# sdu-hpcl/BGSA

Hardware: AMD Instinct MI355X
Metric: GCUPS (cell updates/sec) all-pairs Myers 150bp (higher is better)
Workload: dtype u32

## Files before the change

bgsa_amd/__init__.py:

```python
from __future__ import annotations

import ctypes
import os
import subprocess
from pathlib import Path

import numpy as np

HERE = Path(__file__).resolve().parent
LIB_PATH = Path(os.environ["BGSA_HIP_LIB"]) if os.environ.get("BGSA_HIP_LIB") else HERE / "libbgsa_hip.so"
LIB_AB_PATH = HERE / "libbgsa_hip_ab.so"
INCLUDE = HERE.parent / "include" / "bgsa_hip.h"

ALGO_MYERS, ALGO_BANDED, ALGO_BITPAL = 0, 1, 2
DISTANCE_BEYOND = -2
V_NUM = 64

_lib = None


class Params(ctypes.Structure):
    _fields_ = [("algo", ctypes.c_int), ("alignment", ctypes.c_int), ("match", ctypes.c_int),
                ("mismatch", ctypes.c_int), ("gap", ctypes.c_int), ("k", ctypes.c_int)]

# ... 79 lines not shown
    L.bgsa_hip_bucket_resident.argtypes = [vp, sz, i32]
    L.bgsa_hip_bucket_release.argtypes = [vp]
    u64p = ctypes.POINTER(ctypes.c_uint64)
    L.bgsa_hip_seam_stats.argtypes = [u64p, u64p, u64p]
    L.bgsa_hip_row_cache_stats.argtypes = [u64p, u64p]
    L.bgsa_hip_event_create.argtypes = [ctypes.POINTER(vp)]
    L.bgsa_hip_event_destroy.argtypes = [vp]
    L.bgsa_hip_event_record.argtypes = [vp, vp]
    L.bgsa_hip_event_synchronize.argtypes = [vp]
    L.bgsa_hip_event_elapsed_ms.argtypes = [vp, vp, ctypes.POINTER(ctypes.c_float)]
    L.bgsa_hip_stream_wait_event.argtypes = [vp, vp]
    L.bgsa_hip_query_stream.argtypes = [i32, vp, i32, i32, vp, i32]
    L.bgsa_hip_myers_band_stream.argtypes = [vp, i32, i32, vp, i32]
    L.bgsa_hip_myers_band_half.argtypes = [i32, i32]
    L.bgsa_hip_myers_band_stats.argtypes = [vp, i32]
    L.bgsa_hip_kernel_name.argtypes = [i32, i32]
    L.bgsa_hip_kernel_name.restype = ctypes.c_char_p
    L.bgsa_hip_malloc.argtypes = [ctypes.POINTER(vp), sz]
    L.bgsa_hip_free.argtypes = [vp]
    L.bgsa_hip_malloc_host.argtypes = [ctypes.POINTER(vp), sz]
    L.bgsa_hip_free_host.argtypes = [vp]
    L.bgsa_hip_memcpy_h2d.argtypes = [vp, vp, sz, vp]
    L.bgsa_hip_memcpy_d2h.argtypes = [vp, vp, sz, vp]
    L.bgsa_hip_memset.argtypes = [vp, i32, sz, vp]
    L.bgsa_hip_stream_synchronize.argtypes = [vp]
    L.bgsa_hip_stream_create.argtypes = [ctypes.POINTER(vp)]
    L.bgsa_hip_stream_destroy.argtypes = [vp]
    L.bgsa_hip_set_device.argtypes = [i32]
    L.hip_handle_reads.argtypes = [vp, vp, i32, i64, i64]
    L.hip_handle_reads.restype = None
# ... 544 lines not shown
```

bgsa_amd/csrc/bgsa_common.h:

```cpp
#pragma once

#include <hip/hip_runtime.h>
#include <stdint.h>
#include <stdlib.h>
#include <stdio.h>

#include <type_traits>

#include "../../include/bgsa_hip.h"

namespace bgsa {

constexpr int kLanes = HIP_V_NUM;
constexpr int kChars = BGSA_CHAR_NUM;
constexpr int kWavesPerBlock = 4;
constexpr int kMaxWords = 32;

void set_error(const char *what, hipError_t e, const char *file, int line);
void set_error_text(const char *text);

#define BGSA_HIP_TRY(expr)                                              \
    do {                                                                \
        hipError_t e_ = (expr);                                         \
        if (e_ != hipSuccess) {                                         \
// ... 46 lines not shown
        if (((N == nw ? (rc = f(std::integral_constant<int, N>{}), true) : false) || ...)) return rc;
        char msg[128];
        snprintf(msg, sizeof msg, "%s: no kernel of %d words in this build", family, nw);
        set_error_text(msg);
        return BGSA_HIP_EUNSUPPORTED;
    }
    template <int M>
    constexpr Widths<N..., M> with() const { return {}; }
};
template <typename A, typename B> struct JoinWidths;
template <int... A, int... B> struct JoinWidths<Widths<A...>, Widths<B...>> { using type = Widths<A..., B...>; };
template <typename A, typename B> using Join = typename JoinWidths<A, B>::type;

int launch_myers(const ScoreArgs &a, int semi_global = 0);
const char *myers_kernel_name(int word_num, int semi_global = 0);

constexpr int kCodeEnd = 5, kCodeRefill = 6;
inline int stream_windows(int ref_len) { return ref_len / 7 + 1; }
inline size_t stream_stride(int ref_len) { return static_cast<size_t>(stream_windows(ref_len) + 1) * 8; }
__host__ __device__ inline unsigned long long plain_stream_window(const char *row, int ref_len, int i)
{
    const int n_windows = ref_len / 7 + 1;
    unsigned long long win = 0;
    for (int j = 0; j < 8; j++) {
        unsigned code = kCodeEnd;
        if (i < n_windows) {
            const int pos = 7 * i + j;
            if (j == 7) code = (i < n_windows - 1) ? kCodeRefill : kCodeEnd;
            else if (pos < ref_len) {
                code = static_cast<unsigned char>(row[pos]);
// ... 432 lines not shown
```

bgsa_amd/csrc/capi.hip:

```cpp
#include <stdlib.h>
#include <string.h>

#include <algorithm>
#include <atomic>
#include <chrono>
#include <map>
#include <memory>
#include <mutex>
#include <string>
#include <thread>
#include <utility>
#include <vector>

#include "bgsa_common.h"
#include "myers_band.h"

namespace bgsa {

static thread_local std::string g_last_error;

void set_error(const char *what, hipError_t e, const char *file, int line)
{
    char buf[512];
    snprintf(buf, sizeof buf, "%s failed: %s (%s:%d)", what, hipGetErrorString(e), file, line);
// ... 526 lines not shown
                 (value & BGSA_HIP_FAULT_BUDGET) ? "window budget exhausted before END " : "",
                 (value & BGSA_HIP_FAULT_CODE) ? "byte that is no stream code dispatched " : "",
                 (value & BGSA_HIP_FAULT_PAIR) ? "align_pairs / trace_pairs: query index outside [0, n_queries) " : "",
                 (value & BGSA_HIP_FAULT_BAND) ? "align_pairs_banded: a traceback step left its block's window" : "");
        set_error_text(msg);
    }
    return static_cast<int>(value);
}

int bgsa_hip_myers_band_half(int ref_len, int read_len)
{
    if (ref_len <= 0 || read_len <= 0) return BGSA_HIP_EINVAL;
    BandSchedule s;
    const int h = band_half(ref_len, read_len);
    return band_schedule(ref_len, read_len, h, (read_len + 31) / 32, &s) ? h : 0;
}

int bgsa_hip_myers_band_stream(const char *mapped_row, int ref_len, int read_len, unsigned char *dst, int cap)
{
    if (!mapped_row || ref_len <= 0 || read_len <= 0) return BGSA_HIP_EINVAL;
    BandSchedule s;
    if (!band_schedule(ref_len, read_len, band_half(ref_len, read_len), (read_len + 31) / 32, &s)) return 0;
    const int n = band_stream_layout(ref_len, s, mapped_row, nullptr);
    if (dst && cap >= n)
        for (int i = 0; 8 * i < n; i++) {
            memset(dst + 8 * i, kCodeEnd, 8);
            band_stream_layout(ref_len, s, mapped_row, dst + 8 * i, 8 * i, 8);
        }
    return n;
}
// ... 1134 lines not shown
```

bgsa_amd/csrc/gen_rows_asm.py:

```python
#!/usr/bin/env python3
from __future__ import annotations

import os
import sys
from pathlib import Path

sys.path.insert(0, str(Path(__file__).resolve().parent))
import rows_ir as R

MYERS_NW = [1, 2, 3, 4, 5, 6, 7, 8, 10, 12, 14, 16, 18, 20, 22, 24, 25]
MYERS_PARKED_NW = [18, 26, 28]
MYERS_SPLIT_NW = [30, 32]
MYERS_SPLIT = int(os.environ.get("BGSA_GEN_MYERS_SPLIT", "9"))
MYERS_SEMI_SPLIT_NW = [26, 28, 30, 32]
MYERS_PARK = os.environ.get("BGSA_GEN_MYERS_PARK", "sgpr")
MYERS_ILP = tuple(int(x) for x in os.environ.get("BGSA_GEN_MYERS_ILP", "2,24").split(","))
MYERS_BALANCED = os.environ.get("BGSA_GEN_MYERS_BALANCED", "0") == "1"


def ilp(body: R.Body) -> R.Body:
    return R.schedule_ilp(body, MYERS_ILP[0], MYERS_ILP[1], *MYERS_ILP[2:3]) if MYERS_ILP[0] > 0 else body


def ilp_planes(body: R.Body) -> R.Body:
    return ilp(body) if os.environ.get("BGSA_GEN_MYERS_ILP_PLANES", "0") == "1" else body


MYERS_PLANES_SPLIT = int(os.environ.get("BGSA_GEN_MYERS_PLANES_SPLIT", "0"))
MYERS_PEQ_BLOCK_NW = [12, 14, 16, 18, 20]
MYERS_BAND_NW = list(range(3, R.MYERS_BAND_MAX_WORDS + 1))
MYERS_PAIR_NW = [1, 2]
MYERS_PLANES_NW = [10, 12, 14, 16, 18, 20, 22, 24, 26, 28, 30, 32]
MYERS_SEMI_PLANES_NW = [26, 28, 30, 32]
MYERS_BLOCK_NW = [12, 14, 16, 18, 20, 22, 24, 26, 28]
BITPAL_VGPR_BUDGET = 224
BITPAL_BLOCK_VGPR_BUDGET = 248

S_WIN, S_WIN_LO = "s[60:61]", "s60"
S_NXT = "s[62:63]"
S_BASE_LO, S_BASE_HI = "s64", "s65"
S_PC, S_PC_LO, S_PC_HI = "s[66:67]", "s66", "s67"
S_C = "s68"
S_PTR, S_PTR_LO, S_PTR_HI = "s[70:71]", "s70", "s71"
S_PARK = ["s[72:73]", "s[74:75]"]
S_LEFT = "s69"
# ... 118 lines not shown
                                                   const unsigned long long stream,
                                                   const int n_windows)
{{
    uint32_t tmp[{max(n_slots, 1)}];
    int left;
    asm volatile(
{text}
        : {", ".join(outs)}
        : {", ".join(ins)}
        : {clob});
    return left;
}}
"""


def gen_band_function(nw: int) -> str:
    windows = [(a, b) for a in range(nw) for b in range(a, nw)]
    assert all(R.myers_window_index(nw, a, b) == k for k, (a, b) in enumerate(windows))
    k_full = R.myers_window_index(nw, 0, nw - 1)
    full = ilp(R.myers_body(nw, 1, balanced=MYERS_BALANCED))
    slot_of, n_slots = full.allocate_temps()
    stride = f"(L_g{k_full}s1_%= - L_g{k_full}s0_%=)"

    def reg_for(c: int, slots: dict):
        def reg(name: str) -> str:
            if name.startswith("S"):
                return f"%[s{name[1:]}]"
            if name.startswith("E"):
                return f"%[e{c}_{name[1:]}]"
            return f"%[t{slots[name]}]"
        return reg

    def disp() -> list[str]:
        return [
            f"s_and_b32 {S_C}, {S_WIN_LO}, 7",
# ... 8 lines not shown
        return f".fill ({stride} - (L_g{k}e{s}_%= - L_g{k}s{s}_%=)) / 4, 4, 0xbf800000"

    asm: list[str] = [
        f"s_mov_b64 {S_PTR}, %[qp]",
        f"s_mov_b32 {S_LEFT}, %[nwin]",
        f"s_load_dwordx2 {S_WIN}, {S_PTR}, 0x0",
        f"s_load_dwordx2 {S_NXT}, {S_PTR}, 0x8",
        f"s_getpc_b64 {S_PC}",
        "L_anchor_%=:",
        f"s_add_u32 {S_BASE_LO}, {S_PC_LO}, (L_g{k_full}s0_%= - L_anchor_%=)",
        f"s_addc_u32 {S_BASE_HI}, {S_PC_HI}, 0",
        "s_waitcnt lgkmcnt(0)",
    ]
    asm += disp()
    for k, (a, b) in enumerate(windows):
        body = full if (a, b) == (0, nw - 1) else ilp(R.myers_window_body(nw, a, b, balanced=MYERS_BALANCED))
        slots, n = (slot_of, n_slots) if body is full else body.allocate_temps()
        assert n <= n_slots
        for c in range(5):
            asm.append(f"L_g{k}s{c}_%=:")
            asm += body.emit_asm(reg_for(c, slots), c)
            asm += disp()
            if body is not full:
                asm.append(f"L_g{k}e{c}_%=:")
                asm.append(pad(k, c))
        asm.append(f"L_g{k}s5_%=:")
        asm.append("s_branch L_done_%=")
        asm.append(f"L_g{k}e5_%=:")
        asm.append(pad(k, 5))
        asm.append(f"L_g{k}s6_%=:")
        asm += [
# ... 20 lines not shown
            f"s_getpc_b64 {S_PC}",
            f"L_g{k}a_%=:",
            f"s_sub_u32 {S_PC_LO}, {S_PC_LO}, (L_g{k}a_%= - L_g0s0_%=)",
            f"s_subb_u32 {S_PC_HI}, {S_PC_HI}, 0",
            f"s_add_u32 {S_BASE_LO}, {S_PC_LO}, {S_C}",
            f"s_addc_u32 {S_BASE_HI}, {S_PC_HI}, 0",
        ]
        asm += disp()
        asm.append(f"L_g{k}e7_%=:")
        asm.append(pad(k, 7))
    asm.append("L_fail_%=:")
    asm += fail_slot()
    asm += done()

    text = "\n".join(f'        "{line}\\n\\t"' if not line.endswith(":") else f'        "{line}\\n"' for line in asm)
    outs = [f'[s{i}] "+v"(state[{i}])' for i in range(2 * nw)]
    outs += ['[left] "=s"(left)']
    outs += [f'[t{i}] "=&v"(tmp[{i}])' for i in range(n_slots)]
    ins = [f'[e{c}_{j}] "v"(P[{c}][{j}])' for c in range(5) for j in range(nw)]
    ins += ['[qp] "s"(stream)', '[nwin] "s"(n_windows)', '[band] "s"(band)']
    clob = ", ".join(f'"{c}"' for c in CLOBBERS)
    return f"""
// {len(windows)} windows; full rows {full.valu_count()} VALU, {n_slots} temporaries
template <>
__device__ __forceinline__ int myers_band_rows_asm<{nw}>(uint32_t (&state)[{2 * nw}],
                                                  const uint32_t (&P)[5][{nw}],
                                                  const unsigned long long stream,
                                                  const int n_windows, const int band)
{{
    uint32_t tmp[{n_slots}];
    int left;
    asm volatile(
{text}
        : {", ".join(outs)}
        : {", ".join(ins)}
        : {clob});
    return left;
}}
"""


# ... 1131 lines not shown
        if packed:
            body, init, n_words = R.bitpal_packed_block_body(nw, sc)
            assert len(init) == NC and not any(init) and n_words == NCW
            parts.append(gen_packed_blocked_function("bitpal_packed_block_rows_asm", nw, body, B * nw, n_words, nw))
        else:
            blocked, init = R.bitpal_block_body(nw, sc)
            assert len(init) == NC and not any(init)
            parts.append(gen_blocked_function("bitpal_block_rows_asm", nw, blocked, B * nw, NC, 0, nw))
    return "".join(parts)


def band_inc_text() -> str:
    parts = ["// GENERATED by gen_rows_asm.py --band from rows_ir.py at build time — do not edit.\n",
             "// Certified band (DESIGN §4.2): the rows of one query on the band stream (myers_band.h), each row on the words of its\n"
             "// window only; band = 0: every row on all NW words (the fallback of a wave whose certificate failed).\n"
             "template <int NW>\n"
             "__device__ __forceinline__ int myers_band_rows_asm(uint32_t (&state)[2 * NW],\n"
             "                                                    const uint32_t (&P)[5][NW],\n"
             "                                                    const unsigned long long stream, const int n_windows,\n"
             "                                                    const int band);\n"]
    parts += [gen_band_function(nw) for nw in MYERS_BAND_NW]
    return "".join(parts)


def main() -> int:
    if "--band" in sys.argv:
        Path(sys.argv[sys.argv.index("--band") + 1]).write_text(band_inc_text())
        return 0
    here = Path(sys.argv[sys.argv.index("--out") + 1]) if "--out" in sys.argv else Path(__file__).resolve().parent
    head = "// GENERATED by gen_rows_asm.py from rows_ir.py — do not edit.\n"
    parts = [head,
             "// All rows of one query against the G groups of one wave.  state[(g*NW+w)*2] = VP,\n"
             "// +1 = VN; P[c][g*NW+w] = match mask of character class c; `stream` = device address\n"
             "// (8-byte aligned, wave-uniform) of the packed query stream; n_windows = windows the stream\n"
             "// holds minus one = REFILLs a well-formed stream performs (the loop never does more).\n"
             "template <int NW, int G>\n"
# ... 80 lines not shown
```

bgsa_amd/csrc/myers_global.hip:

```cpp
#include <stdlib.h>
#include <string.h>

#include <algorithm>

#include "bgsa_common.h"
#include "myers_band.h"

namespace bgsa {

template <int NW, int G, bool SEMI = false>
__device__ __forceinline__ void myers_row(uint32_t (&vp)[G * NW], uint32_t (&vn)[G * NW],
                                          const uint32_t (&eq)[G * NW], int last_word = 0, int last_bit = 0,
                                          int *delta = nullptr)
{
#pragma unroll
  for (int gi = 0; gi < G; gi++) {
    uint32_t hp_prev = 0, hn_prev = 0;
    unsigned carry = 0;
#pragma unroll
    for (int ww = 0; ww < NW; ww++) {
        const int w = gi * NW + ww;
        const uint32_t pv = vp[w], mv = vn[w], e = eq[w];
        const uint32_t pm = e | mv;
        unsigned cout;
// ... 83 lines not shown
#pragma unroll
            for (int w = 0; w < NW; w++) {
                const int rem = read_len - 32 * w;
                const uint32_t m = rem >= 32 ? ~0u : (rem <= 0 ? 0u : ((1u << rem) - 1u));
                score += __popc(vp[gi * NW + w] & m) - __popc(vn[gi * NW + w] & m);
            }
            if (group0 + gi < n_groups)
                dst[static_cast<size_t>(q - ref_start) * ld + gi * kLanes] = static_cast<int16_t>(-score);
        }
    }
}

constexpr int kPeqMaxWords = 32;
constexpr int kSemiPeqMaxWords = 32;
constexpr int kPairMaxWords = 2;
#include "myers_rows_gen.inc"
#include "_gen/myers_band_rows_gen.inc"

template <int NW, int G, bool DYN = false, bool BAND = false, bool LENS = false>
__global__ __launch_bounds__(256) void myers_global_asm_kernel(
    const unsigned char *__restrict__ streams, const uint32_t *__restrict__ peq,
    int16_t *__restrict__ out, int ref_len, int read_len, long long ld, int n_groups, int word_num,
    int n_queries, int q_tile, int stream_stride_bytes, unsigned *__restrict__ fault_word,
    unsigned *__restrict__ task_counter, int band_limit = 0, unsigned long long *__restrict__ band_launch = nullptr,
    const int32_t *__restrict__ read_lens = nullptr)
{
    static_assert(!BAND || (G == 1 && NW >= kBandMinWords && NW <= kBandMaxWords), "band: one group, 3..8 words");
    static_assert(!(LENS && BAND), "the certified band is derived from one (m, n): a length-aware launch runs full rows");
    constexpr bool kLenPerQuery = LENS && NW > 8;
    const int lane = threadIdx.x & (kLanes - 1);
    const unsigned wave_groups = (static_cast<unsigned>(n_groups) + G - 1) / G;
    const unsigned n_tasks = wave_groups * ((static_cast<unsigned>(n_queries) + q_tile - 1) / q_tile);
    unsigned task = 0, task_issued = 0;
    if constexpr (DYN) {
        task = first_wave_task();
        if (task >= n_tasks) return;
    }
    int band_on = 1, unreported = 0;
    do {
        int group0, tile;
        if constexpr (DYN) {
            group0 = static_cast<int>((task % wave_groups) * G);
// ... 28 lines not shown
        int16_t *dst = out + static_cast<size_t>(group0) * kLanes + lane;

        for (int q = q0; q < q1; q++) {
            if constexpr (DYN) {
                if (q == q1 - 1) task_issued = issue_wave_task(task_counter);
            }
            uint32_t st[2 * G * NW];
#pragma unroll
            for (int w = 0; w < G * NW; w++) {
                st[2 * w] = ~0u;
                st[2 * w + 1] = 0u;
            }
            const unsigned long long s =
                reinterpret_cast<unsigned long long>(streams) + static_cast<unsigned long long>(q) * stream_stride_bytes;
            if constexpr (BAND) {
                const int tried = band_on;
                int band = band_on, score;
                for (;;) {
                    const int left = myers_band_rows_asm<NW>(st, P, uniform_u64(s),
                                                             __builtin_amdgcn_readfirstlane(stream_stride_bytes / 8 - 2),
                                                             __builtin_amdgcn_readfirstlane(band));
                    note_stream_fault(fault_word, left);
                    score = ref_len;
#pragma unroll
                    for (int w = 0; w < NW; w++) {
                        const int rem = read_len - 32 * w;
                        const uint32_t m = rem >= 32 ? ~0u : (rem <= 0 ? 0u : ((1u << rem) - 1u));
                        score += __popc(st[2 * w] & m) - __popc(st[2 * w + 1] & m);
                    }
                    if (!band || __builtin_amdgcn_ballot_w64(score > band_limit) == 0) break;
                    band = 0;
                    unsigned long long r = 1, b = static_cast<unsigned long long>(unreported) + 1;
                    if (lane == 0) {
                        r += atomicAdd(&band_launch[0], 1ull);
                        b += atomicAdd(&band_launch[1], b);
                    }
                    r = uniform_u64(r);
                    b = uniform_u64(b);
                    unreported = -1;
                    if (b >= 64 && 8 * r > b) band_on = 0;
#pragma unroll
                    for (int w = 0; w < NW; w++) {
                        st[2 * w] = ~0u;
                        st[2 * w + 1] = 0u;
                    }
                }
                unreported += tried;
                dst[static_cast<size_t>(q) * ld] = static_cast<int16_t>(-score);
                continue;
            }
            int left;
            if constexpr (NW <= kPairMaxWords)
                left = myers_pair_rows_asm<NW, G>(st, P, uniform_u64(s), __builtin_amdgcn_readfirstlane(stream_stride_bytes / 8 - 2));
            else
                left = myers_rows_asm<NW, G>(st, P, uniform_u64(s), __builtin_amdgcn_readfirstlane(stream_stride_bytes / 8 - 2));
            note_stream_fault(fault_word, left);
#pragma unroll
            for (int gi = 0; gi < G; gi++) {
                int score = ref_len;
                int n_cols = read_len;
                if constexpr (kLenPerQuery) {
                    unsigned lane_e;
                    asm volatile("v_mbcnt_lo_u32_b32 %0, -1, 0\n\tv_mbcnt_hi_u32_b32 %0, -1, %0" : "=v"(lane_e));
                    n_cols = group0 + gi < n_groups ? lane_read_len(read_lens, static_cast<size_t>(group0 + gi) * kLanes + lane_e, read_len) : 0;
                }
                else if constexpr (LENS)
                    n_cols = own_len[gi];
                if constexpr (LENS) asm volatile("" : "+v"(n_cols));
#pragma unroll
                for (int w = 0; w < NW; w++) {
                    const int rem = n_cols - 32 * w;
                    const uint32_t m = rem >= 32 ? ~0u : (rem <= 0 ? 0u : ((1u << rem) - 1u));
                    score += __popc(st[2 * (gi * NW + w)] & m) - __popc(st[2 * (gi * NW + w) + 1] & m);
                }
                if (group0 + gi < n_groups)
                    dst[static_cast<size_t>(q) * ld + gi * kLanes] = static_cast<int16_t>(-score);
            }
        }
        if constexpr (DYN) task = resolve_wave_task(task_issued);
    } while (DYN && task < n_tasks);
    if constexpr (BAND) {
        if (lane == 0 && unreported) atomicAdd(&band_launch[1], static_cast<unsigned long long>(unreported));
    }
}

__device__ __forceinline__ uint32_t semi_source_word(const uint32_t *row, int word_num, int i)
{
    const int ic = i < 0 ? 0 : (i >= word_num ? word_num - 1 : i);
    return row[ic * kLanes] & ((i >= 0 && i < word_num) ? ~0u : 0u);
}
__device__ __forceinline__ uint32_t semi_funnel(uint32_t hi, uint32_t lo, int r)
// ... 288 lines not shown
                        run += static_cast<int>((hpw >> (31 - b2)) & 1u) - static_cast<int>((hnw >> (31 - b2)) & 1u);
                        best = run < best ? run : best;
                    }
                }
                score = best;
            }
            out[static_cast<size_t>(q) * ld + static_cast<size_t>(group) * kLanes + lane] = static_cast<int16_t>(-score);
        }
    }
}

namespace {

using PeqWidths = Widths<1, 2, 3, 4, 5, 6, 7, 8, 10, 12, 14, 16, 18, 20, 22, 24, 25, 26, 28, 30, 32>;
using PairWidths = Widths<1, 2>;
using PlanesAbWidths = Widths<10, 12, 14, 16, 18, 20, 22, 24, 26, 28>;
using PlanesWidths = Widths<30, 32>;
using SemiPlanesWidths = Widths<26, 28, 30, 32>;
using PeqBlockWidths = Widths<12, 14, 16, 18, 20>;
using PlaneBlockWidths = Widths<12, 14, 16, 18, 20, 22, 24, 26, 28>;
using CompilerWidths = Widths<1, 2, 3, 4, 5, 6, 7, 8, 10, 12, 14, 16, 20, 24, 28, 32>;
static_assert(kPairMaxWords == 2 && kPeqMaxWords == 32 && kSemiPeqMaxWords == 32, "the width lists above restate these");

int pick_q_tile(int nq, int64_t n_wave_tasks, int ref_len, int words)
{
    return pick_query_tile(nq, n_wave_tasks, static_cast<long long>(ref_len) * words, 32);
}

int myers_impl()
{
    static const int impl = [] {
        const char *e = getenv("BGSA_MYERS_IMPL");
        return (e && e[0] == 'c') ? 1 : 0;
    }();
    return impl;
}

static int pair_groups()
{
    static const int g = [] {
        const char *e = getenv("BGSA_MYERS_PAIR_GROUPS");
        return (e && e[0] == '1') ? 1 : 2;
    }();
    return g;
}

static unsigned myers_lds_pad()
{
    static const unsigned v = [] { const char *e = getenv("BGSA_MYERS_LDS_PAD"); return e ? static_cast<unsigned>(atoi(e)) : 0u; }();
    return v;
}

static int long_query_tile()
{
    static const int v = [] {
        const char *e = getenv("BGSA_MYERS_LONG_TILE");
        const int t = e ? atoi(e) : 32;
        return (t == 8 || t == 16 || t == 32) ? t : 32;
    }();
    return v;
// ... 11 lines not shown
__global__ void band_stats_add_kernel(const unsigned long long *__restrict__ launch, unsigned long long *__restrict__ stats)
{
    atomicAdd(&stats[0], launch[0]);
    atomicAdd(&stats[1], launch[1]);
}

using AsmKernel = void (*)(const unsigned char *, const uint32_t *, int16_t *, int, int, long long, int, int, int, int, int,
                           unsigned *, unsigned *, int, unsigned long long *, const int32_t *);

template <int NW, int G>
int launch_asm(const ScoreArgs &a)
{
    const int nq = a.nq();
    constexpr bool kCounter = NW <= 8 || NW >= 30;
    constexpr bool kPairs = NW <= kPairMaxWords;
    const bool lens = a.d_read_lens != nullptr;
    const int64_t n_waves = (a.n_groups() + G - 1) / G;
    const TaskPlan plan = plan_tasks(nq, n_waves, static_cast<long long>(a.ref_len) * NW * G, NW >= 30 ? 8 : 32, kCounter,
                                     NW >= 30 ? long_query_tile() : query_tile_max(), lens);
    if (lens && kCounter && !plan.dynamic) {
        set_error_text("myers: too many tasks for one length-aware launch (split the query window)");
        return BGSA_HIP_EUNSUPPORTED;
    }
    note_query_tile(plan.q_tile);
    AsmKernel on_grid = myers_global_asm_kernel<NW, G, false>, on_counter = nullptr;
    if constexpr (kCounter) on_counter = myers_global_asm_kernel<NW, G, true>;
    if (lens) {
        if constexpr (kCounter) on_grid = nullptr, on_counter = myers_global_asm_kernel<NW, G, true, false, true>;
        else on_grid = myers_global_asm_kernel<NW, G, false, false, true>;
    }
    BandSchedule sched;
    int h = 0;
    bool band = false;
    if constexpr (G == 1 && NW >= kBandMinWords && NW <= kBandMaxWords) {
        h = band_half(a.ref_len, a.read_len);
        band = !lens && band_schedule(a.ref_len, a.read_len, h, NW, &sched);
        if (band) {
            on_grid = myers_global_asm_kernel<NW, G, false, true>;
            on_counter = myers_global_asm_kernel<NW, G, true, true>;
        }
    }
    const int stride = static_cast<int>(band ? band_stream_stride(a.ref_len) : kPairs ? pair_stream_stride(a.ref_len) : stream_stride(a.ref_len));
    unsigned *words = task_counter_in(a.d_workspace, static_cast<size_t>(stride) * nq);
    LaunchGrid lg;
    if (int rc = plan_grid(plan, n_waves, nq, words,
                           [&] { return on_counter ? persistent_blocks_for(on_counter, myers_lds_pad()) : persistent_blocks(); }, "myers", &lg))
        return rc;
    if (int rc = band     ? launch_pack_band(a.d_content, a.ref_len, sched, a.ref_start, a.ref_end, a.d_workspace, a.stream, words)
                 : kPairs ? launch_pack_query_pairs(a.d_content, a.ref_len, a.ref_start, a.ref_end, a.d_workspace, a.stream, lg.counter)
                          : launch_pack_queries(a.d_content, a.ref_len, a.ref_start, a.ref_end, a.d_workspace, a.stream, lg.counter))
        return rc;
    unsigned *fault = nullptr;
    if (int rc = stream_guard(a.d_workspace, stride, kPairs ? kPairRefill : kCodeRefill, band ? kBandBadCode : kPairs ? -1 : 7, a.stream, &fault))
        return rc;
    unsigned long long *guard = band ? band_launch_words(words) : nullptr;
// ... 116 lines not shown
    static const int limit = [] {
        const char *e = getenv("BGSA_MYERS_PEQ_MAX_WORDS");
        const int v = e ? atoi(e) : kPeqMaxWords;
        return (v >= 8 && v <= 32) ? v : kPeqMaxWords;
    }();
    return limit;
}

int myers_semi_max_plain_words() { return 32; }

namespace {

enum class MyersFamily {
    kAsm,
    kAsmPairs,
    kSemiAsm,
    kPlanes,
    kSemiPlanes,
    kBlockedPeq,
    kBlockedPlanes,
    kCompiler,
    kStateInMemory,
};
struct MyersChoice {
    MyersFamily family;
    int nw, G, n_blocks;
    bool semi;
    const char *refused;
};

MyersChoice myers_select(int word_num, int semi, int64_t read_count)
{
    auto ab_only = [](const char *knob) -> const char * { return BGSA_AB_KERNELS ? nullptr : knob; };
    MyersChoice c = {MyersFamily::kAsm, -1, 1, 0, semi != 0, nullptr};
    const bool c_impl = myers_impl() == 1;
    const int peq_max = semi ? std::min(myers_peq_max_words(), kSemiPeqMaxWords) : myers_peq_max_words();
    if (!semi && word_num > myers_max_plain_words()) {
        c.family = peq_blocks() ? MyersFamily::kBlockedPeq : MyersFamily::kBlockedPlanes;
        c.nw = peq_blocks() ? PeqBlockWidths::pick_blocks(word_num, &c.n_blocks) : PlaneBlockWidths::pick_blocks(word_num, &c.n_blocks);
        if (!peq_blocks()) c.refused = ab_only("BGSA_MYERS_BLOCK_FORM=planes");
        if (c_impl) {
            c.family = MyersFamily::kStateInMemory;
            c.refused = ab_only("BGSA_MYERS_IMPL=c");
        }
    } else if (c_impl) {
        c.family = MyersFamily::kCompiler;
        c.nw = CompilerWidths::pick(word_num);
        c.refused = ab_only("BGSA_MYERS_IMPL=c");
    } else if (word_num <= peq_max) {
        c.nw = PeqWidths::pick(word_num);
        if (semi)
            c.family = MyersFamily::kSemiAsm;
        else if (word_num <= kPairMaxWords && pair_groups() == 2 && read_count >= 2 * kLanes) {
            c.family = MyersFamily::kAsmPairs;
            c.G = 2;
        }
    } else if (semi && word_num > myers_semi_max_plain_words()) {
        c.family = MyersFamily::kBlockedPeq;
        c.nw = PeqBlockWidths::pick_blocks(word_num, &c.n_blocks);
    } else if (semi) {
        c.family = MyersFamily::kSemiPlanes;
        c.nw = SemiPlanesWidths::pick(word_num);
    } else {
        c.family = MyersFamily::kPlanes;
        c.nw = Join<PlanesAbWidths, PlanesWidths>::pick(word_num);
        if (!PlanesWidths::has(c.nw)) c.refused = ab_only("BGSA_MYERS_PEQ_MAX_WORDS");
    }
    return c;
}

}

const char *myers_kernel_name(int word_num, int semi_global)
{
    static thread_local char name[64];
    const MyersChoice c = myers_select(word_num, semi_global, 2 * kLanes);
    switch (c.family) {
    case MyersFamily::kAsm:
    case MyersFamily::kAsmPairs: snprintf(name, sizeof name, "myers_global_asm_kernel<%d, %d>", c.nw, c.G); break;
    case MyersFamily::kSemiAsm: snprintf(name, sizeof name, "myers_semi_asm_kernel<%d>", c.nw); break;
    case MyersFamily::kPlanes: snprintf(name, sizeof name, "myers_global_planes_kernel<%d>", c.nw); break;
    case MyersFamily::kSemiPlanes: snprintf(name, sizeof name, "myers_semi_planes_kernel<%d>", c.nw); break;
    case MyersFamily::kStateInMemory:
        snprintf(name, sizeof name, peq_blocks() ? "myers_blocked_kernel<%d, true>" : "myers_blocked_kernel<%d>", c.nw);
        break;
    case MyersFamily::kBlockedPeq: snprintf(name, sizeof name, c.semi ? "myers_blocked_kernel<%d, true, true>" : "myers_blocked_kernel<%d, true>", c.nw); break;
    case MyersFamily::kBlockedPlanes: snprintf(name, sizeof name, "myers_blocked_kernel<%d>", c.nw); break;
    case MyersFamily::kCompiler: snprintf(name, sizeof name, c.semi ? "myers_global_kernel<%d, 1, true>" : "myers_global_kernel<%d, 1>", c.nw); break;
    }
    return name;
}

int launch_myers(const ScoreArgs &a, int semi_global)
{
    if (a.ref_end <= a.ref_start || a.read_count == 0) return BGSA_HIP_OK;
    const MyersChoice c = myers_select(a.word_num, semi_global, a.read_count);
    if (c.refused) return ab_knob_refused(c.refused);
    if (a.d_read_lens && c.family != MyersFamily::kAsm && c.family != MyersFamily::kAsmPairs) {
        set_error_text("myers: per-subject lengths are scored by myers_global_asm_kernel only (global mode, word_num <= 32, no "
                       "BGSA_MYERS_IMPL / BGSA_MYERS_PEQ_MAX_WORDS / BGSA_MYERS_MAX_PLAIN_WORDS alternative)");
        return BGSA_HIP_EUNSUPPORTED;
    }
    switch (c.family) {
    case MyersFamily::kAsm:
        return PeqWidths::dispatch(c.nw, "myers_global_asm_kernel", [&](auto nw) { return launch_asm<decltype(nw)::value, 1>(a); });
    case MyersFamily::kAsmPairs:
        return PairWidths::dispatch(c.nw, "myers_global_asm_kernel (pairs)", [&](auto nw) { return launch_asm<decltype(nw)::value, 2>(a); });
    case MyersFamily::kSemiAsm:
        return PeqWidths::dispatch(c.nw, "myers_semi_asm_kernel", [&](auto nw) { return launch_semi_asm<decltype(nw)::value>(a); });
    case MyersFamily::kPlanes:
        return Join<AbOnly<PlanesAbWidths>, PlanesWidths>::dispatch(c.nw, "myers_global_planes_kernel",
                                                                   [&](auto nw) { return launch_planes<decltype(nw)::value>(a); });
    case MyersFamily::kSemiPlanes:
        return SemiPlanesWidths::dispatch(c.nw, "myers_semi_planes_kernel", [&](auto nw) { return launch_planes<decltype(nw)::value, true>(a); });
    case MyersFamily::kBlockedPeq:
        return PeqBlockWidths::dispatch(c.nw, "myers_blocked_kernel (Peq planes)", [&](auto nw) {
            return c.semi ? launch_blocked<decltype(nw)::value, true, true>(a, c.n_blocks) : launch_blocked<decltype(nw)::value, true>(a, c.n_blocks);
        });
    case MyersFamily::kBlockedPlanes:
        return AbOnly<PlaneBlockWidths>::dispatch(c.nw, "myers_blocked_kernel (code planes)",
                                                  [&](auto nw) { return launch_blocked<decltype(nw)::value>(a, c.n_blocks); });
#if BGSA_AB_KERNELS
// ... 18 lines not shown
```

bgsa_amd/csrc/rows_ir.py:

```python
#!/usr/bin/env python3
from __future__ import annotations

from dataclasses import dataclass, field

import numpy as np


def tt(fn) -> int:
    return fn(0xF0, 0xCC, 0xAA) & 0xFF


TT_XOR3 = tt(lambda a, b, c: a ^ b ^ c)
TT_MAJ = tt(lambda a, b, c: (a & b) | (a & c) | (b & c))
TT_OR3 = tt(lambda a, b, c: a | b | c)
TT_NOR3 = tt(lambda a, b, c: ~(a | b | c))


@dataclass
class Op:
    kind: str
    dst: str = ""
    srcs: tuple = ()
    imm: int = 0
    dst2: str = ""
# ... 448 lines not shown
                if w == hi - 1 and not last and not vg:
                    save(1)
                b.AND(VN(w), M(w), VP(w))
                if w == hi - 1 and not last and not vg:
                    load(0)
                b.BITOP3(VP(w), M(w), A(w), VP(w), lambda m, hn, hp: (m & hn) | ~(m | hp))
                if w == hi - 1 and not last and vg:
                    save(1)
                    load(0)
    return b


MYERS_BAND_MAX_WORDS = 8


def myers_window_body(nw: int, a: int, b: int, balanced: bool = False) -> Body:
    assert 0 <= a <= b < nw
    src = myers_body(b - a + 1, balanced=balanced)

    def ren(x: str) -> str:
        if x.startswith("S"):
            return f"S{int(x[1:]) + 2 * a}"
        if x.startswith("E"):
            return f"E{int(x[1:]) + a}"
        return x

    out = Body()
    out.ops = [Op(op.kind, ren(op.dst), tuple(ren(s) for s in op.srcs), op.imm, op.dst2) for op in src.ops]
    return out


def myers_window_index(nw: int, a: int, b: int) -> int:
    return a * nw - a * (a - 1) // 2 + (b - a)


def myers_band_half(length: int) -> int:
    return (9 * length + 192) // 32


def myers_band_windows(m: int, n: int, h: int, nw: int):
    B = 2 * h + 1
    delta = n - m
    if h <= 0 or abs(delta) > B or nw > MYERS_BAND_MAX_WORDS or nw < 3:
# ... 28 lines not shown
    for i in range(m):
        if win[i] != cur:
            if len(out) % 8 >= 6:
                refill()
            out += bytes([7, myers_window_index(nw, *win[i])])
            cur = win[i]
        put(int(codes[i]))
    put(5)
    while len(out) % 8:
        out.append(5)
    out += bytes([5] * 8)
    return bytes(out)


def run_band_stream(nw: int, state: list, peq: np.ndarray, stream: bytes, band: bool = True, balanced: bool = False,
                    schedule=None) -> int:
    windows = [(a, b) for a in range(nw) for b in range(a, nw)]
    bodies = {}
    cur = (0, nw - 1)
    pos, rows = 0, 0
    while True:
        c = stream[pos]
        if c == 5:
            return rows
        if c == 6:
            pos = (pos | 7) + 1
            continue
        if c == 7:
            k = stream[pos + 1]
            assert k < len(windows) and myers_window_index(nw, *windows[k]) == k
            cur = windows[k] if band else (0, nw - 1)
            pos += 2
            continue
        assert c < 5
        if cur not in bodies:
            bodies[cur] = myers_window_body(nw, *cur, balanced=balanced)
            if schedule is not None:
                bodies[cur] = schedule(bodies[cur])
        bodies[cur].simulate(state, [peq[c, w] for w in range(nw)], cls=c)
        rows += cur[1] - cur[0] + 1
        pos += 1


def myers_body10(nw: int, groups: int = 1) -> Body:
    b = Body()
    for g in range(groups):
        P = lambda w: f"S{(g * nw + w) * 2}"
        M = lambda w: f"S{(g * nw + w) * 2 + 1}"
        E = lambda w: f"E{g * nw + w}"
        D = lambda w: f"d{g}_{w}"
        HP = lambda w: f"hp{g}_{w}"
        HN = lambda w: f"hn{g}_{w}"
        for w in range(nw):
            b.AND(D(w), P(w), E(w))
# ... 1459 lines not shown
```

include/bgsa_hip.h:

```cpp
#ifndef BGSA_HIP_H
#define BGSA_HIP_H

#include <stddef.h>
#include <stdint.h>

#ifdef __cplusplus
extern "C" {
#endif

#define BGSA_CHAR_NUM 5
#define HIP_V_NUM 64
#define HIP_WORD_SIZE 32
#define HIP_BANDED_WORD_SIZE 64
#define HIP_MAX_ERROR 127
typedef uint32_t hip_read_t;
typedef uint32_t hip_data_t;
typedef int16_t hip_write_t;
typedef int8_t hip_banded_write_t;

#ifndef BGSA_HAVE_SEQ_T
#define BGSA_HAVE_SEQ_T
typedef struct _seq_t {
    int len;
    int64_t size;
// ... 172 lines not shown

#define BGSA_HIP_FAULT_BUDGET 1
#define BGSA_HIP_FAULT_CODE 2
#define BGSA_HIP_FAULT_PAIR 4
#define BGSA_HIP_FAULT_BAND 8
int bgsa_hip_stream_faults(int clear);
int bgsa_hip_debug_inject_stream_fault(int kind);

int bgsa_hip_clock_probe_start(int n_probes, unsigned max_ms, void *caller_stream);
int bgsa_hip_clock_probe_stop(double *mhz, int *xcc, int cap, int *n_out, double *seconds);

int bgsa_hip_query_stream(int algo, const char *mapped_row, int ref_len, int k, unsigned char *dst, int cap);

int bgsa_hip_myers_band_stream(const char *mapped_row, int ref_len, int read_len, unsigned char *dst, int cap);
int bgsa_hip_myers_band_half(int ref_len, int read_len);
int bgsa_hip_myers_band_stats(unsigned long long *out, int clear);

int bgsa_hip_last_query_tile(void);

const char *bgsa_hip_kernel_name(int algo, int word_num);

#ifdef __cplusplus
}
#endif
#endif
```

Baseline: 381,700.

## Run the certified Myers band kernel on two subject groups per wave for 3-5 words

Adds a two-group variant of the banded Myers row kernel for 3 to 5 words. Each wave interleaves the bit-vector updates of two 64-subject groups in one generated asm loop, with a wider ILP scheduling window. It is selected automatically when the band certificate holds and the read count is large. The goal is to amortise the per-row stream decode and dispatch over twice the work and to expose more independent instructions. The cost is doubled state and Peq registers, which may lower occupancy. The band fallback now redoes both groups whenever either one exceeds the limit.

```diff
diff --git a/bgsa_amd/__init__.py b/bgsa_amd/__init__.py
--- a/bgsa_amd/__init__.py
+++ b/bgsa_amd/__init__.py
@@ -117,6 +117,8 @@
     L.bgsa_hip_myers_band_stream.argtypes = [vp, i32, i32, vp, i32]
     L.bgsa_hip_myers_band_half.argtypes = [i32, i32]
     L.bgsa_hip_myers_band_stats.argtypes = [vp, i32]
+    if hasattr(L, "bgsa_hip_myers_band_groups"):
+        L.bgsa_hip_myers_band_groups.argtypes = [i32, i64, i32, i32, i32]
     L.bgsa_hip_kernel_name.argtypes = [i32, i32]
     L.bgsa_hip_kernel_name.restype = ctypes.c_char_p
     L.bgsa_hip_malloc.argtypes = [ctypes.POINTER(vp), sz]
diff --git a/bgsa_amd/csrc/bgsa_common.h b/bgsa_amd/csrc/bgsa_common.h
--- a/bgsa_amd/csrc/bgsa_common.h
+++ b/bgsa_amd/csrc/bgsa_common.h
@@ -84,6 +84,7 @@
 
 int launch_myers(const ScoreArgs &a, int semi_global = 0);
 const char *myers_kernel_name(int word_num, int semi_global = 0);
+int myers_band_groups(int word_num, int64_t read_count, int ref_len, int read_len, int mixed_lengths);
 
 constexpr int kCodeEnd = 5, kCodeRefill = 6;
 inline int stream_windows(int ref_len) { return ref_len / 7 + 1; }
diff --git a/bgsa_amd/csrc/capi.hip b/bgsa_amd/csrc/capi.hip
--- a/bgsa_amd/csrc/capi.hip
+++ b/bgsa_amd/csrc/capi.hip
@@ -564,6 +564,12 @@
     BandSchedule s;
     const int h = band_half(ref_len, read_len);
     return band_schedule(ref_len, read_len, h, (read_len + 31) / 32, &s) ? h : 0;
+}
+
+int bgsa_hip_myers_band_groups(int word_num, int64_t read_count, int ref_len, int read_len, int mixed_lengths)
+{
+    if (word_num <= 0 || read_count < 0 || ref_len <= 0 || read_len <= 0) return BGSA_HIP_EINVAL;
+    return myers_band_groups(word_num, read_count, ref_len, read_len, mixed_lengths);
 }
 
 int bgsa_hip_myers_band_stream(const char *mapped_row, int ref_len, int read_len, unsigned char *dst, int cap)
diff --git a/bgsa_amd/csrc/gen_rows_asm.py b/bgsa_amd/csrc/gen_rows_asm.py
--- a/bgsa_amd/csrc/gen_rows_asm.py
+++ b/bgsa_amd/csrc/gen_rows_asm.py
@@ -29,6 +29,8 @@
 MYERS_PLANES_SPLIT = int(os.environ.get("BGSA_GEN_MYERS_PLANES_SPLIT", "0"))
 MYERS_PEQ_BLOCK_NW = [12, 14, 16, 18, 20]
 MYERS_BAND_NW = list(range(3, R.MYERS_BAND_MAX_WORDS + 1))
+MYERS_BAND_PAIR_NW = [3, 4, 5]
+MYERS_BAND_PAIR_WINDOW = int(os.environ.get("BGSA_GEN_MYERS_BAND_PAIR_WINDOW", "8"))
 MYERS_PAIR_NW = [1, 2]
 MYERS_PLANES_NW = [10, 12, 14, 16, 18, 20, 22, 24, 26, 28, 30, 32]
 MYERS_SEMI_PLANES_NW = [26, 28, 30, 32]
@@ -177,11 +179,17 @@
 """
 
 
-def gen_band_function(nw: int) -> str:
+def gen_band_function(nw: int, groups: int = 1) -> str:
     windows = [(a, b) for a in range(nw) for b in range(a, nw)]
     assert all(R.myers_window_index(nw, a, b) == k for k, (a, b) in enumerate(windows))
     k_full = R.myers_window_index(nw, 0, nw - 1)
-    full = ilp(R.myers_body(nw, 1, balanced=MYERS_BALANCED))
+    def sched(body: R.Body) -> R.Body:
+        if groups == 1:
+            return ilp(body)
+        return R.schedule_ilp(body, MYERS_ILP[0], MYERS_BAND_PAIR_WINDOW, *MYERS_ILP[2:3]) if MYERS_ILP[0] > 0 else body
+
+    full = sched(R.myers_body(nw, 1, balanced=MYERS_BALANCED) if groups == 1 else
+                 R.myers_window_body(nw, 0, nw - 1, groups=groups, balanced=MYERS_BALANCED))
     slot_of, n_slots = full.allocate_temps()
     stride = f"(L_g{k_full}s1_%= - L_g{k_full}s0_%=)"
 
@@ -220,7 +228,7 @@
     ]
     asm += disp()
     for k, (a, b) in enumerate(windows):
-        body = full if (a, b) == (0, nw - 1) else ilp(R.myers_window_body(nw, a, b, balanced=MYERS_BALANCED))
+        body = full if (a, b) == (0, nw - 1) else sched(R.myers_window_body(nw, a, b, groups=groups, balanced=MYERS_BALANCED))
         slots, n = (slot_of, n_slots) if body is full else body.allocate_temps()
         assert n <= n_slots
         for c in range(5):
@@ -271,17 +279,17 @@
     asm += done()
 
     text = "\n".join(f'        "{line}\\n\\t"' if not line.endswith(":") else f'        "{line}\\n"' for line in asm)
-    outs = [f'[s{i}] "+v"(state[{i}])' for i in range(2 * nw)]
+    outs = [f'[s{i}] "+v"(state[{i}])' for i in range(2 * groups * nw)]
     outs += ['[left] "=s"(left)']
     outs += [f'[t{i}] "=&v"(tmp[{i}])' for i in range(n_slots)]
-    ins = [f'[e{c}_{j}] "v"(P[{c}][{j}])' for c in range(5) for j in range(nw)]
+    ins = [f'[e{c}_{j}] "v"(P[{c}][{j}])' for c in range(5) for j in range(groups * nw)]
     ins += ['[qp] "s"(stream)', '[nwin] "s"(n_windows)', '[band] "s"(band)']
     clob = ", ".join(f'"{c}"' for c in CLOBBERS)
     return f"""
 // {len(windows)} windows; full rows {full.valu_count()} VALU, {n_slots} temporaries
 template <>
-__device__ __forceinline__ int myers_band_rows_asm<{nw}>(uint32_t (&state)[{2 * nw}],
-                                                  const uint32_t (&P)[5][{nw}],
+__device__ __forceinline__ int myers_band_rows_asm<{nw}, {groups}>(uint32_t (&state)[{2 * groups * nw}],
+                                                  const uint32_t (&P)[5][{groups * nw}],
                                                   const unsigned long long stream,
                                                   const int n_windows, const int band)
 {{
@@ -1443,12 +1451,14 @@
     parts = ["// GENERATED by gen_rows_asm.py --band from rows_ir.py at build time — do not edit.\n",
              "// Certified band (DESIGN §4.2): the rows of one query on the band stream (myers_band.h), each row on the words of its\n"
              "// window only; band = 0: every row on all NW words (the fallback of a wave whose certificate failed).\n"
-             "template <int NW>\n"
-             "__device__ __forceinline__ int myers_band_rows_asm(uint32_t (&state)[2 * NW],\n"
-             "                                                    const uint32_t (&P)[5][NW],\n"
+             "// G = 2 (3..5 words): the same loop on two subject groups per wave, state[(g*NW+w)*2] and P[c][g*NW+w] as myers_rows_asm.\n"
+             "template <int NW, int G>\n"
+             "__device__ __forceinline__ int myers_band_rows_asm(uint32_t (&state)[2 * G * NW],\n"
+             "                                                    const uint32_t (&P)[5][G * NW],\n"
              "                                                    const unsigned long long stream, const int n_windows,\n"
              "                                                    const int band);\n"]
     parts += [gen_band_function(nw) for nw in MYERS_BAND_NW]
+    parts += [gen_band_function(nw, 2) for nw in MYERS_BAND_PAIR_NW]
     return "".join(parts)
 
 
diff --git a/bgsa_amd/csrc/myers_global.hip b/bgsa_amd/csrc/myers_global.hip
--- a/bgsa_amd/csrc/myers_global.hip
+++ b/bgsa_amd/csrc/myers_global.hip
@@ -121,6 +121,7 @@
 constexpr int kPeqMaxWords = 32;
 constexpr int kSemiPeqMaxWords = 32;
 constexpr int kPairMaxWords = 2;
+constexpr int kBandPairMaxWords = 5;
 #include "myers_rows_gen.inc"
 #include "_gen/myers_band_rows_gen.inc"
 
@@ -132,7 +133,8 @@
     unsigned *__restrict__ task_counter, int band_limit = 0, unsigned long long *__restrict__ band_launch = nullptr,
     const int32_t *__restrict__ read_lens = nullptr)
 {
-    static_assert(!BAND || (G == 1 && NW >= kBandMinWords && NW <= kBandMaxWords), "band: one group, 3..8 words");
+    static_assert(!BAND || (NW >= kBandMinWords && NW <= kBandMaxWords && (G == 1 || (G == 2 && NW <= kBandPairMaxWords))),
+                  "band: 3..8 words, one subject group per wave — or two up to 5 words");
     static_assert(!(LENS && BAND), "the certified band is derived from one (m, n): a length-aware launch runs full rows");
     constexpr bool kLenPerQuery = LENS && NW > 8;
     const int lane = threadIdx.x & (kLanes - 1);
@@ -191,67 +193,80 @@
             const unsigned long long s =
                 reinterpret_cast<unsigned long long>(streams) + static_cast<unsigned long long>(q) * stream_stride_bytes;
             if constexpr (BAND) {
-                const int tried = band_on;
-                int band = band_on, score;
+                const int n_live = G == 1 ? 1 : (group0 + 1 < n_groups ? 2 : 1);
+                const int tried = band_on * n_live;
+                int band = band_on, score[G];
                 for (;;) {
-                    const int left = myers_band_rows_asm<NW>(st, P, uniform_u64(s),
-                                                             __builtin_amdgcn_readfirstlane(stream_stride_bytes / 8 - 2),
-                                                             __builtin_amdgcn_readfirstlane(band));
+                    const int left = myers_band_rows_asm<NW, G>(st, P, uniform_u64(s),
+                                                                __builtin_amdgcn_readfirstlane(stream_stride_bytes / 8 - 2),
+                                                                __builtin_amdgcn_readfirstlane(band));
                     note_stream_fault(fault_word, left);
-                    score = ref_len;
-#pragma unroll
-                    for (int w = 0; w < NW; w++) {
-                        const int rem = read_len - 32 * w;
-                        const uint32_t m = rem >= 32 ? ~0u : (rem <= 0 ? 0u : ((1u << rem) - 1u));
-                        score += __popc(st[2 * w] & m) - __popc(st[2 * w + 1] & m);
+#pragma unroll
+                    for (int gi = 0; gi < G; gi++) {
+                        score[gi] = ref_len;
+#pragma unroll
+                        for (int w = 0; w < NW; w++) {
+                            const int rem = read_len - 32 * w;
+                            const uint32_t m = rem >= 32 ? ~0u : (rem <= 0 ? 0u : ((1u << rem) - 1u));
+                            score[gi] += __popc(st[2 * (gi * NW + w)] & m) - __popc(st[2 * (gi * NW + w) + 1] & m);
+                        }
                     }
-                    if (!band || __builtin_amdgcn_ballot_w64(score > band_limit) == 0) break;
+                    if (!band) break;
+                    int n_over = 0;
+#pragma unroll
+                    for (int gi = 0; gi < G; gi++)
+                        if (gi < n_live && __builtin_amdgcn_ballot_w64(score[gi] > band_limit) != 0) n_over++;
+                    if (n_over == 0) break;
+                    if constexpr (G == 1) n_over = 1;
                     band = 0;
-                    unsigned long long r = 1, b = static_cast<unsigned long long>(unreported) + 1;
+                    unsigned long long r = static_cast<unsigned long long>(n_over),
+                                       b = static_cast<unsigned long long>(unreported) + n_live;
                     if (lane == 0) {
-                        r += atomicAdd(&band_launch[0], 1ull);
+                        r += atomicAdd(&band_launch[0], r);
                         b += atomicAdd(&band_launch[1], b);
                     }
                     r = uniform_u64(r);
                     b = uniform_u64(b);
-                    unreported = -1;
+                    unreported = -n_live;
                     if (b >= 64 && 8 * r > b) band_on = 0;
 #pragma unroll
-                    for (int w = 0; w < NW; w++) {
+                    for (int w = 0; w < G * NW; w++) {
                         st[2 * w] = ~0u;
                         st[2 * w + 1] = 0u;
                     }
                 }
                 unreported += tried;
-                dst[static_cast<size_t>(q) * ld] = static_cast<int16_t>(-score);
-                continue;
-            }
-            int left;
-            if constexpr (NW <= kPairMaxWords)
-                left = myers_pair_rows_asm<NW, G>(st, P, uniform_u64(s), __builtin_amdgcn_readfirstlane(stream_stride_bytes / 8 - 2));
-            else
-                left = myers_rows_asm<NW, G>(st, P, uniform_u64(s), __builtin_amdgcn_readfirstlane(stream_stride_bytes / 8 - 2));
-            note_stream_fault(fault_word, left);
-#pragma unroll
-            for (int gi = 0; gi < G; gi++) {
-                int score = ref_len;
-                int n_cols = read_len;
-                if constexpr (kLenPerQuery) {
-                    unsigned lane_e;
-                    asm volatile("v_mbcnt_lo_u32_b32 %0, -1, 0\n\tv_mbcnt_hi_u32_b32 %0, -1, %0" : "=v"(lane_e));
-                    n_cols = group0 + gi < n_groups ? lane_read_len(read_lens, static_cast<size_t>(group0 + gi) * kLanes + lane_e, read_len) : 0;
+#pragma unroll
+                for (int gi = 0; gi < G; gi++)
+                    if (gi < n_live) dst[static_cast<size_t>(q) * ld + gi * kLanes] = static_cast<int16_t>(-score[gi]);
+            } else {
+                int left;
+                if constexpr (NW <= kPairMaxWords)
+                    left = myers_pair_rows_asm<NW, G>(st, P, uniform_u64(s), __builtin_amdgcn_readfirstlane(stream_stride_bytes / 8 - 2));
+                else
+                    left = myers_rows_asm<NW, G>(st, P, uniform_u64(s), __builtin_amdgcn_readfirstlane(stream_stride_bytes / 8 - 2));
+                note_stream_fault(fault_word, left);
+#pragma unroll
+                for (int gi = 0; gi < G; gi++) {
+                    int score = ref_len;
+                    int n_cols = read_len;
+                    if constexpr (kLenPerQuery) {
+                        unsigned lane_e;
+                        asm volatile("v_mbcnt_lo_u32_b32 %0, -1, 0\n\tv_mbcnt_hi_u32_b32 %0, -1, %0" : "=v"(lane_e));
+                        n_cols = group0 + gi < n_groups ? lane_read_len(read_lens, static_cast<size_t>(group0 + gi) * kLanes + lane_e, read_len) : 0;
+                    }
+                    else if constexpr (LENS)
+                        n_cols = own_len[gi];
+                    if constexpr (LENS) asm volatile("" : "+v"(n_cols));
+#pragma unroll
+                    for (int w = 0; w < NW; w++) {
+                        const int rem = n_cols - 32 * w;
+                        const uint32_t m = rem >= 32 ? ~0u : (rem <= 0 ? 0u : ((1u << rem) - 1u));
+                        score += __popc(st[2 * (gi * NW + w)] & m) - __popc(st[2 * (gi * NW + w) + 1] & m);
+                    }
+                    if (group0 + gi < n_groups)
+                        dst[static_cast<size_t>(q) * ld + gi * kLanes] = static_cast<int16_t>(-score);
                 }
-                else if constexpr (LENS)
-                    n_cols = own_len[gi];
-                if constexpr (LENS) asm volatile("" : "+v"(n_cols));
-#pragma unroll
-                for (int w = 0; w < NW; w++) {
-                    const int rem = n_cols - 32 * w;
-                    const uint32_t m = rem >= 32 ? ~0u : (rem <= 0 ? 0u : ((1u << rem) - 1u));
-                    score += __popc(st[2 * (gi * NW + w)] & m) - __popc(st[2 * (gi * NW + w) + 1] & m);
-                }
-                if (group0 + gi < n_groups)
-                    dst[static_cast<size_t>(q) * ld + gi * kLanes] = static_cast<int16_t>(-score);
             }
         }
         if constexpr (DYN) task = resolve_wave_task(task_issued);
@@ -570,13 +585,14 @@
 
 using PeqWidths = Widths<1, 2, 3, 4, 5, 6, 7, 8, 10, 12, 14, 16, 18, 20, 22, 24, 25, 26, 28, 30, 32>;
 using PairWidths = Widths<1, 2>;
+using BandPairWidths = Widths<3, 4, 5>;
 using PlanesAbWidths = Widths<10, 12, 14, 16, 18, 20, 22, 24, 26, 28>;
 using PlanesWidths = Widths<30, 32>;
 using SemiPlanesWidths = Widths<26, 28, 30, 32>;
 using PeqBlockWidths = Widths<12, 14, 16, 18, 20>;
 using PlaneBlockWidths = Widths<12, 14, 16, 18, 20, 22, 24, 26, 28>;
 using CompilerWidths = Widths<1, 2, 3, 4, 5, 6, 7, 8, 10, 12, 14, 16, 20, 24, 28, 32>;
-static_assert(kPairMaxWords == 2 && kPeqMaxWords == 32 && kSemiPeqMaxWords == 32, "the width lists above restate these");
+static_assert(kPairMaxWords == 2 && kBandPairMaxWords == 5 && kPeqMaxWords == 32 && kSemiPeqMaxWords == 32, "the width lists above restate these");
 
 int pick_q_tile(int nq, int64_t n_wave_tasks, int ref_len, int words)
 {
@@ -600,6 +616,16 @@
     }();
     return g;
 }
+
+static int band_groups_knob()
+{
+    static const int g = [] {
+        const char *e = getenv("BGSA_MYERS_BAND_GROUPS");
+        return (e && (e[0] == '1' || e[0] == '2') && e[1] == 0) ? e[0] - '0' : 0;
+    }();
+    return g;
+}
+constexpr int64_t kBandPairMinReads = 125000;
 
 static unsigned myers_lds_pad()
 {
@@ -641,6 +667,8 @@
     const int nq = a.nq();
     constexpr bool kCounter = NW <= 8 || NW >= 30;
     constexpr bool kPairs = NW <= kPairMaxWords;
+    constexpr bool kBandPair = G == 2 && !kPairs;
+    static_assert(!kBandPair || NW <= kBandPairMaxWords, "two groups per wave: the pair kernels, or the band up to 5 words");
     const bool lens = a.d_read_lens != nullptr;
     const int64_t n_waves = (a.n_groups() + G - 1) / G;
     const TaskPlan plan = plan_tasks(nq, n_waves, static_cast<long long>(a.ref_len) * NW * G, NW >= 30 ? 8 : 32, kCounter,
@@ -650,22 +678,29 @@
         return BGSA_HIP_EUNSUPPORTED;
     }
     note_query_tile(plan.q_tile);
-    AsmKernel on_grid = myers_global_asm_kernel<NW, G, false>, on_counter = nullptr;
-    if constexpr (kCounter) on_counter = myers_global_asm_kernel<NW, G, true>;
-    if (lens) {
-        if constexpr (kCounter) on_grid = nullptr, on_counter = myers_global_asm_kernel<NW, G, true, false, true>;
-        else on_grid = myers_global_asm_kernel<NW, G, false, false, true>;
+    AsmKernel on_grid = nullptr, on_counter = nullptr;
+    if constexpr (!kBandPair) {
+        on_grid = myers_global_asm_kernel<NW, G, false>;
+        if constexpr (kCounter) on_counter = myers_global_asm_kernel<NW, G, true>;
+        if (lens) {
+            if constexpr (kCounter) on_grid = nullptr, on_counter = myers_global_asm_kernel<NW, G, true, false, true>;
+            else on_grid = myers_global_asm_kernel<NW, G, false, false, true>;
+        }
     }
     BandSchedule sched;
     int h = 0;
     bool band = false;
-    if constexpr (G == 1 && NW >= kBandMinWords && NW <= kBandMaxWords) {
+    if constexpr ((G == 1 || kBandPair) && NW >= kBandMinWords && NW <= kBandMaxWords) {
         h = band_half(a.ref_len, a.read_len);
         band = !lens && band_schedule(a.ref_len, a.read_len, h, NW, &sched);
         if (band) {
             on_grid = myers_global_asm_kernel<NW, G, false, true>;
             on_counter = myers_global_asm_kernel<NW, G, true, true>;
         }
+    }
+    if (kBandPair && !band) {
+        set_error_text("myers: two subject groups per wave selected for a launch without the certified band");
+        return BGSA_HIP_EUNSUPPORTED;
     }
     const int stride = static_cast<int>(band ? band_stream_stride(a.ref_len) : kPairs ? pair_stream_stride(a.ref_len) : stream_stride(a.ref_len));
     unsigned *words = task_counter_in(a.d_workspace, static_cast<size_t>(stride) * nq);
@@ -812,6 +847,7 @@
 enum class MyersFamily {
     kAsm,
     kAsmPairs,
+    kAsmBandPairs,
     kSemiAsm,
     kPlanes,
     kSemiPlanes,
@@ -827,7 +863,16 @@
     const char *refused;
 };
 
-MyersChoice myers_select(int word_num, int semi, int64_t read_count)
+int band_groups_for(int nw, int64_t read_count, int ref_len, int read_len, bool mixed_lengths)
+{
+    if (nw < kBandMinWords || nw > kBandPairMaxWords || mixed_lengths || read_count < 2 * kLanes || ref_len <= 0 || read_len <= 0) return 1;
+    BandSchedule sched;
+    if (!band_schedule(ref_len, read_len, band_half(ref_len, read_len), nw, &sched)) return 1;
+    if (band_groups_knob()) return band_groups_knob();
+    return read_count >= kBandPairMinReads ? 2 : 1;
+}
+
+MyersChoice myers_select(int word_num, int semi, int64_t read_count, int ref_len = 0, int read_len = 0, bool mixed_lengths = false)
 {
     auto ab_only = [](const char *knob) -> const char * { return BGSA_AB_KERNELS ? nullptr : knob; };
     MyersChoice c = {MyersFamily::kAsm, -1, 1, 0, semi != 0, nullptr};
@@ -852,6 +897,9 @@
         else if (word_num <= kPairMaxWords && pair_groups() == 2 && read_count >= 2 * kLanes) {
             c.family = MyersFamily::kAsmPairs;
             c.G = 2;
+        } else if (band_groups_for(c.nw, read_count, ref_len, read_len, mixed_lengths) == 2) {
+            c.family = MyersFamily::kAsmBandPairs;
+            c.G = 2;
         }
     } else if (semi && word_num > myers_semi_max_plain_words()) {
         c.family = MyersFamily::kBlockedPeq;
@@ -869,12 +917,20 @@
 
 }
 
+int myers_band_groups(int word_num, int64_t read_count, int ref_len, int read_len, int mixed_lengths)
+{
+    if (word_num < 1 || word_num > kMaxWords) return 1;
+    const MyersChoice c = myers_select(word_num, 0, read_count, ref_len, read_len, mixed_lengths != 0);
+    return c.family == MyersFamily::kAsmBandPairs ? 2 : 1;
+}
+
 const char *myers_kernel_name(int word_num, int semi_global)
 {
     static thread_local char name[64];
     const MyersChoice c = myers_select(word_num, semi_global, 2 * kLanes);
     switch (c.family) {
     case MyersFamily::kAsm:
+    case MyersFamily::kAsmBandPairs:
     case MyersFamily::kAsmPairs: snprintf(name, sizeof name, "myers_global_asm_kernel<%d, %d>", c.nw, c.G); break;
     case MyersFamily::kSemiAsm: snprintf(name, sizeof name, "myers_semi_asm_kernel<%d>", c.nw); break;
     case MyersFamily::kPlanes: snprintf(name, sizeof name, "myers_global_planes_kernel<%d>", c.nw); break;
@@ -892,7 +948,7 @@
 int launch_myers(const ScoreArgs &a, int semi_global)
 {
     if (a.ref_end <= a.ref_start || a.read_count == 0) return BGSA_HIP_OK;
-    const MyersChoice c = myers_select(a.word_num, semi_global, a.read_count);
+    const MyersChoice c = myers_select(a.word_num, semi_global, a.read_count, a.ref_len, a.read_len, a.d_read_lens != nullptr);
     if (c.refused) return ab_knob_refused(c.refused);
     if (a.d_read_lens && c.family != MyersFamily::kAsm && c.family != MyersFamily::kAsmPairs) {
         set_error_text("myers: per-subject lengths are scored by myers_global_asm_kernel only (global mode, word_num <= 32, no "
@@ -904,6 +960,8 @@
         return PeqWidths::dispatch(c.nw, "myers_global_asm_kernel", [&](auto nw) { return launch_asm<decltype(nw)::value, 1>(a); });
     case MyersFamily::kAsmPairs:
         return PairWidths::dispatch(c.nw, "myers_global_asm_kernel (pairs)", [&](auto nw) { return launch_asm<decltype(nw)::value, 2>(a); });
+    case MyersFamily::kAsmBandPairs:
+        return BandPairWidths::dispatch(c.nw, "myers_global_asm_kernel (band, two groups)", [&](auto nw) { return launch_asm<decltype(nw)::value, 2>(a); });
     case MyersFamily::kSemiAsm:
         return PeqWidths::dispatch(c.nw, "myers_semi_asm_kernel", [&](auto nw) { return launch_semi_asm<decltype(nw)::value>(a); });
     case MyersFamily::kPlanes:
diff --git a/bgsa_amd/csrc/rows_ir.py b/bgsa_amd/csrc/rows_ir.py
--- a/bgsa_amd/csrc/rows_ir.py
+++ b/bgsa_amd/csrc/rows_ir.py
@@ -486,19 +486,21 @@
 MYERS_BAND_MAX_WORDS = 8
 
 
-def myers_window_body(nw: int, a: int, b: int, balanced: bool = False) -> Body:
-    assert 0 <= a <= b < nw
+def myers_window_body(nw: int, a: int, b: int, groups: int = 1, balanced: bool = False) -> Body:
+    assert 0 <= a <= b < nw and groups >= 1
     src = myers_body(b - a + 1, balanced=balanced)
-
-    def ren(x: str) -> str:
-        if x.startswith("S"):
-            return f"S{int(x[1:]) + 2 * a}"
-        if x.startswith("E"):
-            return f"E{int(x[1:]) + a}"
-        return x
-
     out = Body()
-    out.ops = [Op(op.kind, ren(op.dst), tuple(ren(s) for s in op.srcs), op.imm, op.dst2) for op in src.ops]
+    for g in range(groups):
+        def ren(x: str) -> str:
+            if x.startswith("S"):
+                return f"S{int(x[1:]) + 2 * (g * nw + a)}"
+            if x.startswith("E"):
+                return f"E{int(x[1:]) + g * nw + a}"
+            if g and x and not x.startswith("$"):
+                return f"{x[0]}{g}{x[2:]}"
+            return x
+
+        out.ops += [Op(op.kind, ren(op.dst), tuple(ren(s) for s in op.srcs), op.imm, op.dst2) for op in src.ops]
     return out
 
 
@@ -557,7 +559,7 @@
 
 
 def run_band_stream(nw: int, state: list, peq: np.ndarray, stream: bytes, band: bool = True, balanced: bool = False,
-                    schedule=None) -> int:
+                    schedule=None, groups: int = 1) -> int:
     windows = [(a, b) for a in range(nw) for b in range(a, nw)]
     bodies = {}
     cur = (0, nw - 1)
@@ -577,10 +579,10 @@
             continue
         assert c < 5
         if cur not in bodies:
-            bodies[cur] = myers_window_body(nw, *cur, balanced=balanced)
+            bodies[cur] = myers_window_body(nw, *cur, groups=groups, balanced=balanced)
             if schedule is not None:
                 bodies[cur] = schedule(bodies[cur])
-        bodies[cur].simulate(state, [peq[c, w] for w in range(nw)], cls=c)
+        bodies[cur].simulate(state, [peq[c, w] for w in range(groups * nw)], cls=c)
         rows += cur[1] - cur[0] + 1
         pos += 1
 
diff --git a/include/bgsa_hip.h b/include/bgsa_hip.h
--- a/include/bgsa_hip.h
+++ b/include/bgsa_hip.h
@@ -210,6 +210,7 @@
 
 int bgsa_hip_myers_band_stream(const char *mapped_row, int ref_len, int read_len, unsigned char *dst, int cap);
 int bgsa_hip_myers_band_half(int ref_len, int read_len);
+int bgsa_hip_myers_band_groups(int word_num, int64_t read_count, int ref_len, int read_len, int mixed_lengths);
 int bgsa_hip_myers_band_stats(unsigned long long *out, int clear);
 
 int bgsa_hip_last_query_tile(void);
```

Result: faster. 391,500 (median of 6 runs) (+2.6%).
